# JohnLonginotto/uq

Measured on AMD Instinct MI355X. Metric: FASTQ encode MB/s (150bp synthetic; bit-exact tables vs reference), higher is better.
Workload: dtype u8

## Files before the change

uq_amd/csrc/index.hip:

```cpp
#include "common.h"
#include "swar.h"

namespace {
constexpr int IDX_THREADS = 256;
constexpr int IDX_LOADS = 4;
constexpr uint64_t IDX_WAVE_BYTES = 64 * 16 * IDX_LOADS;
constexpr uint64_t IDX_TILE = IDX_WAVE_BYTES * (IDX_THREADS / 64);
constexpr uint64_t IDX_TILE_VECS = IDX_TILE / 16;
constexpr uint32_t IDX_LIST_CAP = 1024;
constexpr uint32_t IDX_BUCKET = 1024;

__global__ __launch_bounds__(IDX_THREADS) void count_newlines_kernel(const uint4* __restrict__ abuf, uint32_t mis,
                                                                      uint64_t nbytes, uint64_t nvec,
                                                                      uint32_t* __restrict__ partials, uint16_t* __restrict__ bitmap) {
    __shared__ uint32_t lds[IDX_THREADS / 64];
    const uint32_t lane = lane_id(), w = threadIdx.x >> 6;
    const uint64_t v0 = ((uint64_t)blockIdx.x * IDX_TILE + (uint64_t)w * IDX_WAVE_BYTES) / 16 + lane;
    uint32_t c = 0;
    uint4 q[IDX_LOADS];
#pragma unroll
    for (int it = 0; it < IDX_LOADS; ++it) { const uint64_t vi = v0 + (uint64_t)it * 64; q[it] = abuf[vi < nvec ? vi : nvec - 1]; }
#pragma unroll
    for (int it = 0; it < IDX_LOADS; ++it) {
        uint64_t vi = v0 + (uint64_t)it * 64;
        int64_t p = (int64_t)(vi * 16) - (int64_t)mis;
        const uint32_t m = vi < nvec ? nl_mask16(q[it]) & valid_mask16(p, nbytes) : 0u;
        bitmap[vi] = (uint16_t)m;
        c += __popc(m);
    }
    c = wave_sum(c);
    if (lane == 0) lds[w] = c;
    __syncthreads();
    if (threadIdx.x == 0) partials[blockIdx.x] = lds[0] + lds[1] + lds[2] + lds[3];
}

#ifndef CENSUS_TPW
#define CENSUS_TPW 2
#endif
template <int TPW>
__global__ __launch_bounds__(IDX_THREADS) void census_list_kernel(const uint4* __restrict__ abuf, uint32_t mis, uint64_t nbytes, uint64_t nvec,
                                                                   uint32_t* __restrict__ partials, uint16_t* __restrict__ list,
                                                                   uint32_t* __restrict__ overflow, uint64_t tile0, uint64_t tile_end) {
    __shared__ uint32_t lds[2][IDX_THREADS / 64];
    const uint32_t lane = lane_id(), w = threadIdx.x >> 6;
    uint64_t tile = tile0 + (uint64_t)blockIdx.x * TPW;
    auto request = [&](uint64_t tl, uint4 (&q)[IDX_LOADS]) {
        const uint64_t v0 = (tl * IDX_TILE + (uint64_t)w * IDX_WAVE_BYTES) / 16 + lane;
#pragma unroll
        for (int it = 0; it < IDX_LOADS; ++it) { const uint64_t vi = v0 + (uint64_t)it * 64; q[it] = abuf[vi < nvec ? vi : nvec - 1]; }
    };
    uint4 q[IDX_LOADS];
    request(tile, q);
    bool over = false;
#pragma unroll
    for (int turn = 0; turn < TPW; ++turn, ++tile) {
        if (tile >= tile_end) break;
        uint4 qn[IDX_LOADS];
        if (turn + 1 < TPW && tile + 1 < tile_end) request(tile + 1, qn);
        const uint64_t v0 = (tile * IDX_TILE + (uint64_t)w * IDX_WAVE_BYTES) / 16 + lane;
        uint32_t m[IDX_LOADS];
#pragma unroll
        for (int it = 0; it < IDX_LOADS; ++it) {
            const uint64_t vi = v0 + (uint64_t)it * 64;
            const int64_t p = (int64_t)(vi * 16) - (int64_t)mis;
            m[it] = vi < nvec ? nl_mask16(q[it]) & valid_mask16(p, nbytes) : 0u;
        }
        const uint32_t c0 = __popc(m[0]), c1 = __popc(m[1]), c2 = __popc(m[2]), c3 = __popc(m[3]);
        const uint32_t i01 = wave_inclusive_sum(c0 | (c1 << 16)), i23 = wave_inclusive_sum(c2 | (c3 << 16));
        const uint32_t t01 = __shfl(i01, 63, 64), t23 = __shfl(i23, 63, 64);
        const uint32_t T0 = t01 & 0xFFFFu, T1 = t01 >> 16, T2 = t23 & 0xFFFFu, T3 = t23 >> 16;
        uint32_t* l = lds[turn & 1];
        if (lane == 0) l[w] = T0 + T1 + T2 + T3;
        __syncthreads();
        uint32_t base = 0, total = 0;
#pragma unroll
        for (uint32_t i = 0; i < IDX_THREADS / 64; ++i) { const uint32_t x = l[i]; if (i < w) base += x; total += x; }
        if (threadIdx.x == 0) partials[tile] = total;
        const uint32_t ex[IDX_LOADS] = {base + (i01 & 0xFFFFu) - c0, base + T0 + (i01 >> 16) - c1, base + T0 + T1 + (i23 & 0xFFFFu) - c2,
                                        base + T0 + T1 + T2 + (i23 >> 16) - c3};
        uint16_t* slot = list + tile * IDX_LIST_CAP;
#pragma unroll
        for (int it = 0; it < IDX_LOADS; ++it) {
            uint32_t mm = m[it], k = ex[it];
            const uint32_t pos0 = ((w * IDX_LOADS + it) * 64 + lane) * 16;
            while (mm) {
                const uint32_t b = (uint32_t)__ffs((int)mm) - 1u;
                mm &= mm - 1;
                if (k < IDX_LIST_CAP) slot[k] = (uint16_t)(pos0 + b); else over = true;
                ++k;
            }
        }
        if (turn + 1 < TPW) {
#pragma unroll
            for (int it = 0; it < IDX_LOADS; ++it) q[it] = qn[it];
        }
    }
    if (over) atomicOr(overflow, 1u);
}

__global__ __launch_bounds__(IDX_THREADS) void census_bucket_kernel(const uint32_t* __restrict__ partials, uint64_t nb, uint32_t* __restrict__ buckets) {
    __shared__ uint32_t lds[IDX_THREADS / 64];
    const uint64_t i0 = (uint64_t)blockIdx.x * IDX_BUCKET + (uint64_t)threadIdx.x * 4;
    uint32_t s = 0;
#pragma unroll
    for (uint32_t k = 0; k < 4; ++k) s += i0 + k < nb ? partials[i0 + k] : 0u;
    s = wave_sum(s);
    if (lane_id() == 0) lds[threadIdx.x >> 6] = s;
    __syncthreads();
    if (threadIdx.x == 0) buckets[blockIdx.x] = lds[0] + lds[1] + lds[2] + lds[3];
}
__global__ __launch_bounds__(IDX_THREADS) void census_scan_kernel(uint32_t* __restrict__ partials, uint64_t nb, const uint32_t* __restrict__ buckets,
                                                                   unsigned long long* __restrict__ d_async) {
    __shared__ uint32_t lds[IDX_THREADS / 64 + 1];
    static_assert(IDX_BUCKET == 4 * IDX_THREADS, "four counts a lane");
    const uint32_t b = blockIdx.x;
    uint32_t s = 0;
    for (uint32_t i = threadIdx.x; i < b; i += IDX_THREADS) s += buckets[i];
    s = wave_sum(s);
    if (lane_id() == 0) lds[threadIdx.x >> 6] = s;
    __syncthreads();
    uint32_t base = 0;
#pragma unroll
    for (uint32_t i = 0; i < IDX_THREADS / 64; ++i) base += lds[i];
    __syncthreads();
    const uint64_t i0 = (uint64_t)b * IDX_BUCKET + (uint64_t)threadIdx.x * 4;
    uint32_t v[4], sum = 0;
#pragma unroll
    for (uint32_t k = 0; k < 4; ++k) { v[k] = i0 + k < nb ? partials[i0 + k] : 0u; sum += v[k]; }
    uint32_t tot;
    uint32_t run = base + block_exclusive_sum<uint32_t, IDX_THREADS / 64>(sum, lds, tot);
#pragma unroll
    for (uint32_t k = 0; k < 4; ++k) { if (i0 + k < nb) partials[i0 + k] = run; run += v[k]; }
    if (b == gridDim.x - 1 && threadIdx.x == 0) d_async[0] = (unsigned long long)(base + tot);
}

__global__ void census_clear_kernel(uint32_t* __restrict__ region, uint32_t nwords, unsigned long long* __restrict__ d_async) {
    const uint32_t i = blockIdx.x * blockDim.x + threadIdx.x;
    if (i < nwords) region[i] = 0;
    if (i < 8) d_async[i] = 0;
}

constexpr uint32_t EXP_TILES = 4;
__global__ __launch_bounds__(IDX_THREADS) void expand_list_kernel(const uint16_t* __restrict__ list, uint32_t mis, const uint32_t* __restrict__ offsets,
                                                                   uint64_t nb, uint64_t nlines, uint64_t* __restrict__ line_start,
                                                                   unsigned long long* __restrict__ d_async, uint64_t cap,
                                                                   const uint32_t* __restrict__ d_over) {
    const uint32_t lane = lane_id();
    const uint64_t tile0 = ((uint64_t)blockIdx.x * (IDX_THREADS / 64) + (threadIdx.x >> 6)) * EXP_TILES;
    if (tile0 >= nb) return;
    if (d_async) nlines = d_async[0];
    if (tile0 == 0 && lane == 0) line_start[0] = 0;
    if (d_async && *d_over) { if (lane == 0) d_async[1] = 1ull; return; }
    const uint64_t tl = tile0 + lane;
    const uint64_t mine = lane <= EXP_TILES ? (tl < nb ? (uint64_t)offsets[tl] : nlines) : 0;
    for (uint32_t k = 0; k < EXP_TILES && tile0 + k < nb; ++k) {
        const uint64_t tile = tile0 + k;
        const uint64_t P = __shfl(mine, k, 64), end = __shfl(mine, k + 1, 64);
        uint32_t cnt = (uint32_t)(end - P);
        const uint16_t* slot = list + tile * IDX_LIST_CAP;
        const int64_t p0 = (int64_t)(tile * IDX_TILE) - (int64_t)mis + 1;
        if (cnt > IDX_LIST_CAP) {
            if (d_async && lane == 0) d_async[1] = 1ull;
            cnt = IDX_LIST_CAP;
        }
        if (d_async && end > cap) {
            if (lane == 0) d_async[1] = 1ull;
            for (uint32_t j = lane; j < cnt; j += 64) if (P + j + 1 <= cap) line_start[P + j + 1] = (uint64_t)(p0 + slot[j]);
            continue;
        }
        for (uint32_t j = lane; j < cnt; j += 64) line_start[P + j + 1] = (uint64_t)(p0 + slot[j]);
    }
}

__global__ __launch_bounds__(IDX_THREADS) void scatter_newlines_kernel(const uint64_t* __restrict__ bitmap, uint32_t mis,
                                                                        const uint32_t* __restrict__ offsets,
                                                                        uint64_t nlines, uint64_t* __restrict__ line_start) {
    __shared__ uint32_t lds[IDX_THREADS / 64 + 1];
    const uint64_t wi = (uint64_t)blockIdx.x * IDX_THREADS + threadIdx.x;
    uint64_t m = bitmap[wi];
    const uint32_t c = (uint32_t)__popcll(m);
    uint32_t total;
    const uint32_t ex = block_exclusive_sum<uint32_t, IDX_THREADS / 64>(c, lds, total);
    if (blockIdx.x == 0 && threadIdx.x == 0) line_start[0] = 0;
    uint64_t k = (uint64_t)offsets[blockIdx.x] + ex;
    const int64_t p = (int64_t)(wi * 64) - (int64_t)mis;
    while (m) {
        const int b = __ffsll((unsigned long long)m) - 1;
        m &= m - 1;
        if (++k <= nlines) line_start[k] = (uint64_t)(p + b + 1);
    }
}

int census_buffers(uq_ctx* ctx, uint64_t nb) {
    if (nb + 1 > ctx->idx_partials_cap) {
        UQ_CHECK_HIP(hipStreamSynchronize(ctx->stream));
        if (ctx->idx_partials) UQ_CHECK_HIP(hipFree(ctx->idx_partials));
        if (ctx->idx_bitmap) UQ_CHECK_HIP(hipFree(ctx->idx_bitmap));
        ctx->idx_partials = nullptr; ctx->idx_bitmap = nullptr; ctx->idx_partials_cap = 0;
        UQ_CHECK_HIP(hipMalloc((void**)&ctx->idx_partials, (nb + 1) * sizeof(uint32_t)));
        static_assert(IDX_TILE_VECS == IDX_LIST_CAP, "bitmap words and list entries per tile share one allocation");
        UQ_CHECK_HIP(hipMalloc((void**)&ctx->idx_bitmap, nb * IDX_TILE_VECS * sizeof(uint16_t) + 16 + ((nb + IDX_BUCKET - 1) / IDX_BUCKET) * sizeof(uint32_t)));
        ctx->idx_partials_cap = nb + 1;
    }
    return 0;
}

uint32_t* census_buckets(uq_ctx* ctx, uint64_t nb) { return (uint32_t*)(ctx->idx_bitmap + nb * IDX_TILE_VECS) + 4; }

int run_count(uq_ctx* ctx, const uint8_t* d_buf, uint64_t nbytes, uint64_t* nblocks_out, bool list_form) {
    const uint32_t mis = (uint32_t)((uintptr_t)d_buf & 15);
    const uint64_t nvec = (nbytes + mis + 15) / 16;
    const uint64_t nb = (nvec * 16 + IDX_TILE - 1) / IDX_TILE;
    UQ_REQUIRE(nb <= 0x7fffffffu, "uq_count_lines: buffer too large for one launch");
    ctx->async_buf = nullptr;
    ctx->census_begun = false;
    UQ_TRY(census_buffers(ctx, nb));
    if (list_form) {
        uint32_t* d_over = (uint32_t*)(ctx->idx_bitmap + nb * IDX_TILE_VECS);
        UQ_CHECK_HIP(hipMemsetAsync(d_over, 0, 4, ctx->stream));
        census_list_kernel<CENSUS_TPW><<<(uint32_t)((nb + CENSUS_TPW - 1) / CENSUS_TPW), IDX_THREADS, 0, ctx->stream>>>((const uint4*)(d_buf - mis), mis, nbytes, nvec, ctx->idx_partials,
                                                                         ctx->idx_bitmap, d_over, 0, nb);
    } else {
        count_newlines_kernel<<<(uint32_t)nb, IDX_THREADS, 0, ctx->stream>>>((const uint4*)(d_buf - mis), mis, nbytes, nvec, ctx->idx_partials,
                                                                            ctx->idx_bitmap);
    }
    UQ_LAUNCH_CHECK();
    *nblocks_out = nb;
    return 0;
}
}

static int finish_count(uq_ctx* ctx, const uint8_t* d_buf, uint64_t nbytes, uint64_t nb, uint64_t* h_nlines);

extern "C" int uq_count_lines(uq_ctx* ctx, const uint8_t* d_buf, uint64_t nbytes, uint64_t* h_nlines) {
    UQ_REQUIRE(ctx && h_nlines, "uq_count_lines: null argument");
    ctx->idx_buf = nullptr;
    if (nbytes == 0) { *h_nlines = 0; return 0; }
    UQ_REQUIRE(d_buf, "uq_count_lines: null buffer");
    uint64_t nb;
    UQ_TRY(run_count(ctx, d_buf, nbytes, &nb, true));
    return finish_count(ctx, d_buf, nbytes, nb, h_nlines);
}

static int finish_count(uq_ctx* ctx, const uint8_t* d_buf, uint64_t nbytes, uint64_t nb, uint64_t* h_nlines) {
    ctx->census_begun = false;
    void* scr;
    UQ_TRY(uq_scratch(ctx, 256, &scr));
    UQ_TRY(uq_scan_exclusive_u32(ctx, ctx->idx_partials, ctx->idx_partials, nb, (uint64_t*)scr));
    UQ_TRY(uq_read_back(ctx, ctx->h_pinned, scr, 8));
    UQ_TRY(uq_read_back(ctx, ctx->h_pinned + 1, ctx->idx_bitmap + nb * IDX_TILE_VECS, 4));
    UQ_CHECK_HIP(hipStreamSynchronize(ctx->stream));
    *h_nlines = ctx->h_pinned[0];
    if ((uint32_t)ctx->h_pinned[1] == 0) { ctx->idx_buf = d_buf; ctx->idx_nbytes = nbytes; ctx->idx_nlines = *h_nlines; }
    return 0;
}

extern "C" int uq_count_lines_begin(uq_ctx* ctx, const uint8_t* d_buf, uint64_t nbytes) {
    UQ_REQUIRE(ctx && (d_buf || nbytes == 0), "uq_count_lines_begin: null argument");
    ctx->census_begun = false;
    ctx->idx_buf = nullptr;
    ctx->async_buf = nullptr;
    if (nbytes == 0) return 0;
    const uint32_t mis = (uint32_t)((uintptr_t)d_buf & 15);
    const uint64_t nb = (((nbytes + mis + 15) / 16) * 16 + IDX_TILE - 1) / IDX_TILE;
    UQ_REQUIRE(nb <= 0x7fffffffu, "uq_count_lines_begin: buffer too large");
    UQ_TRY(census_buffers(ctx, nb));
    census_clear_kernel<<<1, 64, 0, ctx->stream>>>((uint32_t*)(ctx->idx_bitmap + nb * IDX_TILE_VECS), 4, ctx->d_async);
    UQ_LAUNCH_CHECK();
    ctx->census_begun = true; ctx->census_nb = nb;
    return 0;
}

extern "C" int uq_count_lines_chunk(uq_ctx* ctx, const uint8_t* d_buf, uint64_t nbytes, uint64_t first_byte, uint64_t chunk_bytes) {
    UQ_REQUIRE(ctx && d_buf, "uq_count_lines_chunk: null argument");
    if (chunk_bytes == 0) return 0;
    const uint32_t mis = (uint32_t)((uintptr_t)d_buf & 15);
    const uint64_t nvec = (nbytes + mis + 15) / 16;
    const uint64_t nb = (nvec * 16 + IDX_TILE - 1) / IDX_TILE;
    UQ_REQUIRE(first_byte + chunk_bytes <= nbytes, "uq_count_lines_chunk: chunk beyond the buffer");
    UQ_REQUIRE((first_byte + mis) % IDX_TILE == 0 || first_byte == 0, "uq_count_lines_chunk: a chunk must start on a 16 KiB tile boundary");
    UQ_REQUIRE((first_byte + chunk_bytes + mis) % IDX_TILE == 0 || first_byte + chunk_bytes == nbytes,
               "uq_count_lines_chunk: a chunk must end on a 16 KiB tile boundary or with the buffer");
    const uint64_t t0 = (first_byte + mis) / IDX_TILE, t1 = first_byte + chunk_bytes == nbytes ? nb : (first_byte + chunk_bytes + mis) / IDX_TILE;
    if (t1 <= t0) return 0;
    census_list_kernel<CENSUS_TPW><<<(uint32_t)((t1 - t0 + CENSUS_TPW - 1) / CENSUS_TPW), IDX_THREADS, 0, ctx->stream>>>((const uint4*)(d_buf - mis), mis, nbytes, nvec, ctx->idx_partials,
                                                                            ctx->idx_bitmap, (uint32_t*)(ctx->idx_bitmap + nb * IDX_TILE_VECS), t0, t1);
    UQ_LAUNCH_CHECK();
    return 0;
}

extern "C" int uq_count_lines_end(uq_ctx* ctx, const uint8_t* d_buf, uint64_t nbytes, uint64_t* h_nlines) {
    UQ_REQUIRE(ctx && h_nlines, "uq_count_lines_end: null argument");
    if (nbytes == 0) { *h_nlines = 0; return 0; }
    const uint32_t mis = (uint32_t)((uintptr_t)d_buf & 15);
    const uint64_t nb = (((nbytes + mis + 15) / 16) * 16 + IDX_TILE - 1) / IDX_TILE;
    return finish_count(ctx, d_buf, nbytes, nb, h_nlines);
}

extern "C" int uq_count_lines_end_async(uq_ctx* ctx, const uint8_t* d_buf, uint64_t nbytes) {
    UQ_REQUIRE(ctx && (d_buf || nbytes == 0), "uq_count_lines_end_async: null argument");
    ctx->idx_buf = nullptr; ctx->async_buf = nullptr; ctx->async_read = false;
    const bool begun = ctx->census_begun && nbytes != 0;
    ctx->census_begun = false;
    if (!begun) UQ_CHECK_HIP(hipMemsetAsync(ctx->d_async, 0, 64, ctx->stream));
    if (nbytes == 0) { ctx->h_pinned[8000] = 0; ctx->h_pinned[8001] = 0; ctx->h_pinned[8002] = 0; ctx->async_buf = d_buf; ctx->async_nbytes = 0; return 0; }
    const uint32_t mis = (uint32_t)((uintptr_t)d_buf & 15);
    const uint64_t nb = (((nbytes + mis + 15) / 16) * 16 + IDX_TILE - 1) / IDX_TILE;
    if (begun && ctx->census_nb == nb) {
        const uint32_t nbk = (uint32_t)((nb + IDX_BUCKET - 1) / IDX_BUCKET);
        census_bucket_kernel<<<nbk, IDX_THREADS, 0, ctx->stream>>>(ctx->idx_partials, nb, census_buckets(ctx, nb));
        UQ_LAUNCH_CHECK();
        census_scan_kernel<<<nbk, IDX_THREADS, 0, ctx->stream>>>(ctx->idx_partials, nb, census_buckets(ctx, nb), ctx->d_async);
        UQ_LAUNCH_CHECK();
    } else {
        if (begun) UQ_CHECK_HIP(hipMemsetAsync(ctx->d_async, 0, 64, ctx->stream));
        UQ_TRY(uq_scan_exclusive_u32(ctx, ctx->idx_partials, ctx->idx_partials, nb, (uint64_t*)ctx->d_async));
    }
    ctx->async_buf = d_buf; ctx->async_nbytes = nbytes;
    return 0;
}

extern "C" int uq_index_lines_async(uq_ctx* ctx, const uint8_t* d_buf, uint64_t nbytes, uint64_t capacity_lines, uint64_t* d_line_start) {
    UQ_REQUIRE(ctx && d_line_start, "uq_index_lines_async: null argument");
    UQ_REQUIRE(ctx->async_buf == d_buf && ctx->async_nbytes == nbytes, "uq_index_lines_async: not the buffer of the last uq_count_lines_end_async");
    UQ_REQUIRE(capacity_lines < (uint64_t(1) << 32), "uq_index_lines_async: more than 2^32-1 lines in one shard");
    if (nbytes == 0) { UQ_CHECK_HIP(hipMemsetAsync(d_line_start, 0, 8, ctx->stream)); return 0; }
    const uint32_t mis = (uint32_t)((uintptr_t)d_buf & 15);
    const uint64_t nb = (((nbytes + mis + 15) / 16) * 16 + IDX_TILE - 1) / IDX_TILE;
    expand_list_kernel<<<(uint32_t)((nb + EXP_TILES * (IDX_THREADS / 64) - 1) / (EXP_TILES * (IDX_THREADS / 64))), IDX_THREADS, 0, ctx->stream>>>(ctx->idx_bitmap, mis, ctx->idx_partials,
                                                                                                                 nb, 0, d_line_start, ctx->d_async, capacity_lines,
                                                                                                                 (const uint32_t*)(ctx->idx_bitmap + nb * IDX_TILE_VECS));
    UQ_LAUNCH_CHECK();
    return 0;
}

namespace {
__global__ void async_read_back_kernel(const uint32_t* __restrict__ d_async, const uint32_t* __restrict__ over, uint32_t* __restrict__ dst) {
    const uint32_t t = threadIdx.x;
    if (t < 4) dst[t] = d_async[t];
    else if (t == 4) dst[4] = *over;
}
}

bool uq_async_sources(uq_ctx* ctx, const uint32_t** d_async, const uint32_t** d_over) {
    if (!ctx->async_buf || ctx->async_nbytes == 0 || ctx->async_read) return false;
    const uint32_t mis = (uint32_t)((uintptr_t)ctx->async_buf & 15);
    const uint64_t nb = (((ctx->async_nbytes + mis + 15) / 16) * 16 + IDX_TILE - 1) / IDX_TILE;
    *d_async = (const uint32_t*)ctx->d_async; *d_over = (const uint32_t*)(ctx->idx_bitmap + nb * IDX_TILE_VECS);
    return true;
}

int uq_async_read_back(uq_ctx* ctx) {
    const uint32_t *d_async, *d_over;
    if (!uq_async_sources(ctx, &d_async, &d_over)) return 0;
    async_read_back_kernel<<<1, 64, 0, ctx->stream>>>(d_async, d_over, (uint32_t*)(ctx->d_pinned + 8000));
    UQ_LAUNCH_CHECK();
    ctx->async_read = true;
    return 0;
}

extern "C" int uq_count_lines_wait(uq_ctx* ctx, const uint8_t* d_buf, uint64_t nbytes, uint64_t* h_nlines, int* h_ok) {
    UQ_REQUIRE(ctx && h_nlines && h_ok, "uq_count_lines_wait: null argument");
    UQ_REQUIRE(ctx->async_buf == d_buf && ctx->async_nbytes == nbytes, "uq_count_lines_wait: not the buffer of the last uq_count_lines_end_async");
    *h_nlines = 0; *h_ok = 1;
    if (nbytes == 0) { ctx->async_buf = nullptr; return 0; }
    UQ_TRY(uq_async_read_back(ctx));
    ctx->async_read = false;
    ctx->async_buf = nullptr;
    UQ_CHECK_HIP(hipStreamSynchronize(ctx->stream));
    *h_nlines = ctx->h_pinned[8000];
    *h_ok = ctx->h_pinned[8001] == 0 && (uint32_t)ctx->h_pinned[8002] == 0;
    return 0;
}

extern "C" int uq_index_lines(uq_ctx* ctx, const uint8_t* d_buf, uint64_t nbytes, uint64_t nlines, uint64_t* d_line_start) {
    UQ_REQUIRE(ctx && d_line_start, "uq_index_lines: null argument");
    UQ_REQUIRE(nlines < (uint64_t(1) << 32), "uq_index_lines: more than 2^32-1 lines in one shard");
    if (nbytes == 0 || nlines == 0) {
        UQ_CHECK_HIP(hipMemsetAsync(d_line_start, 0, 8, ctx->stream));
        return 0;
    }
    uint64_t nb;
    const uint32_t mis = (uint32_t)((uintptr_t)d_buf & 15);
    const uint64_t nvec = (nbytes + mis + 15) / 16;
    if (ctx->idx_buf == d_buf && ctx->idx_nbytes == nbytes) {
        UQ_REQUIRE(ctx->idx_nlines == nlines, "uq_index_lines: nlines %llu does not match the census %llu",
                   (unsigned long long)nlines, (unsigned long long)ctx->idx_nlines);
        nb = (nvec * 16 + IDX_TILE - 1) / IDX_TILE;
        ctx->idx_buf = nullptr;
        expand_list_kernel<<<(uint32_t)((nb + EXP_TILES * (IDX_THREADS / 64) - 1) / (EXP_TILES * (IDX_THREADS / 64))), IDX_THREADS, 0, ctx->stream>>>(ctx->idx_bitmap, mis, ctx->idx_partials,
                                                                                                                     nb, nlines, d_line_start, nullptr, 0, nullptr);
        UQ_LAUNCH_CHECK();
        return 0;
    }
    UQ_TRY(run_count(ctx, d_buf, nbytes, &nb, false));
    UQ_TRY(uq_scan_exclusive_u32(ctx, ctx->idx_partials, ctx->idx_partials, nb, nullptr));
    ctx->idx_buf = nullptr;
    scatter_newlines_kernel<<<(uint32_t)nb, IDX_THREADS, 0, ctx->stream>>>((const uint64_t*)ctx->idx_bitmap, mis, ctx->idx_partials, nlines,
                                                                           d_line_start);
    UQ_LAUNCH_CHECK();
    return 0;
}
```

uq_amd/csrc/swar.h:

```cpp
#pragma once
#include "common.h"

__device__ __forceinline__ uint32_t nl_bits(uint32_t v) {
    v ^= 0x0A0A0A0Au;
    uint32_t t = (v & 0x7F7F7F7Fu) + 0x7F7F7F7Fu;
    return ~(t | v | 0x7F7F7F7Fu);
}
__device__ __forceinline__ uint32_t nl_mask16(uint4 q) {
    auto nib = [](uint32_t w) { return (((nl_bits(w) >> 7) & 0x01010101u) * 0x01020408u >> 24) & 0xFu; };
    return nib(q.x) | (nib(q.y) << 4) | (nib(q.z) << 8) | (nib(q.w) << 12);
}
__device__ __forceinline__ uint32_t valid_mask16(int64_t p, uint64_t nbytes) {
    if (p >= 0 && (uint64_t)p + 16 <= nbytes) return 0xFFFFu;
    uint32_t m = 0;
#pragma unroll
    for (int i = 0; i < 16; ++i) {
        int64_t q = p + i;
        if (q >= 0 && (uint64_t)q < nbytes) m |= 1u << i;
    }
    return m;
}

__device__ __forceinline__ void lds_window8(const uint8_t* base, int32_t o, uint32_t& lo, uint32_t& hi) {
    const uint32_t* p = (const uint32_t*)(base + (o & ~3));
    const uint32_t a = p[0], b = p[1], c = p[2];
    const uint32_t sh = (uint32_t)o & 3u;
    lo = __builtin_amdgcn_alignbyte(b, a, sh);
    hi = __builtin_amdgcn_alignbyte(c, b, sh);
}
__device__ __forceinline__ void lds_window8_at(const uint8_t* base, int32_t aligned, uint32_t sh, uint32_t& lo, uint32_t& hi) {
    const uint32_t* p = (const uint32_t*)(base + aligned);
    const uint32_t a = p[0], b = p[1], c = p[2];
    lo = __builtin_amdgcn_alignbyte(b, a, sh);
    hi = __builtin_amdgcn_alignbyte(c, b, sh);
}
__device__ __forceinline__ void window_masks(uint32_t nbad, uint32_t& mlo, uint32_t& mhi) {
    mlo = nbad >= 4 ? 0u : (0xFFFFFFFFu << (8 * nbad));
    mhi = nbad >= 8 ? 0u : (nbad > 4 ? (0xFFFFFFFFu << (8 * (nbad - 4))) : 0xFFFFFFFFu);
}
__device__ __forceinline__ uint32_t bfi(uint32_t mask, uint32_t a, uint32_t b) { return (a & mask) | (b & ~mask); }
__device__ __forceinline__ uint32_t nonzero_bytes(uint32_t x) {
    const uint32_t nz = (((x & 0x7F7F7F7Fu) + 0x7F7F7F7Fu) | x) & 0x80808080u;
    return (nz - (nz >> 7)) | nz;
}
```

Before: 1.628 million.

## Rework census list kernel: one tile per block, LDS-staged list, DPP scan

The census list kernel now handles one tile per block instead of two prefetched tiles. Loads are nontemporal with a clamped in-tile index, and newline masks come from udot4 byte packing. Per-byte validity masking is confined to edge tiles, and the wave prefix sum uses DPP. Newline positions are written as scattered 16-bit stores into an LDS image, then copied out to global memory with coalesced 16-byte stores. The aim is to cut scattered global writes and ALU work, at the cost of an extra barrier and losing the cross-tile load prefetch.

```diff
diff --git a/uq_amd/csrc/index.hip b/uq_amd/csrc/index.hip
--- a/uq_amd/csrc/index.hip
+++ b/uq_amd/csrc/index.hip
@@ -34,68 +34,79 @@
     if (threadIdx.x == 0) partials[blockIdx.x] = lds[0] + lds[1] + lds[2] + lds[3];
 }
 
-#ifndef CENSUS_TPW
-#define CENSUS_TPW 2
-#endif
-template <int TPW>
-__global__ __launch_bounds__(IDX_THREADS) void census_list_kernel(const uint4* __restrict__ abuf, uint32_t mis, uint64_t nbytes, uint64_t nvec,
-                                                                   uint32_t* __restrict__ partials, uint16_t* __restrict__ list,
-                                                                   uint32_t* __restrict__ overflow, uint64_t tile0, uint64_t tile_end) {
-    __shared__ uint32_t lds[2][IDX_THREADS / 64];
+__device__ __forceinline__ uint32_t wave_inclusive_sum_dpp(uint32_t x) {
+    int v = (int)x;
+    v += __builtin_amdgcn_update_dpp(0, v, 0x111, 0xf, 0xf, false);
+    v += __builtin_amdgcn_update_dpp(0, v, 0x112, 0xf, 0xf, false);
+    v += __builtin_amdgcn_update_dpp(0, v, 0x114, 0xf, 0xf, false);
+    v += __builtin_amdgcn_update_dpp(0, v, 0x118, 0xf, 0xf, false);
+    v += __builtin_amdgcn_update_dpp(0, v, 0x142, 0xa, 0xf, false);
+    v += __builtin_amdgcn_update_dpp(0, v, 0x143, 0xc, 0xf, false);
+    return (uint32_t)v;
+}
+
+__global__ __launch_bounds__(IDX_THREADS, 8) void census_list_kernel(const uint4* __restrict__ abuf, uint32_t mis, uint64_t nbytes, uint64_t nvec,
+                                                                      uint32_t* __restrict__ partials, uint16_t* __restrict__ list,
+                                                                      uint32_t* __restrict__ overflow, uint64_t tile0) {
+    __shared__ uint32_t lds[IDX_THREADS / 64];
+    __shared__ __attribute__((aligned(16))) uint16_t img[IDX_LIST_CAP];
     const uint32_t lane = lane_id(), w = threadIdx.x >> 6;
-    uint64_t tile = tile0 + (uint64_t)blockIdx.x * TPW;
-    auto request = [&](uint64_t tl, uint4 (&q)[IDX_LOADS]) {
-        const uint64_t v0 = (tl * IDX_TILE + (uint64_t)w * IDX_WAVE_BYTES) / 16 + lane;
-#pragma unroll
-        for (int it = 0; it < IDX_LOADS; ++it) { const uint64_t vi = v0 + (uint64_t)it * 64; q[it] = abuf[vi < nvec ? vi : nvec - 1]; }
-    };
+    const uint32_t off = w * (uint32_t)(IDX_WAVE_BYTES / 16) + lane;
+    const uint64_t tl = tile0 + blockIdx.x;
+    const char* src = (const char*)(abuf + tl * IDX_TILE_VECS);
+    const uint64_t left = nvec - tl * IDX_TILE_VECS;
+    const uint32_t last = left < IDX_TILE_VECS ? (uint32_t)left - 1u : (uint32_t)IDX_TILE_VECS - 1u;
     uint4 q[IDX_LOADS];
-    request(tile, q);
+#pragma unroll
+    for (int it = 0; it < IDX_LOADS; ++it) {
+        typedef uint32_t v4u __attribute__((ext_vector_type(4)));
+        const v4u x = __builtin_nontemporal_load((const v4u*)(src + min(off + (uint32_t)it * 64u, last) * 16u));
+        q[it] = make_uint4(x.x, x.y, x.z, x.w);
+    }
+    uint32_t m[IDX_LOADS];
+#pragma unroll
+    for (int it = 0; it < IDX_LOADS; ++it) m[it] = nl_mask16_dot(q[it]);
+    if (!((tl > 0 || mis == 0) && (tl + 1) * IDX_TILE <= nbytes + mis)) {
+        const uint64_t room = nbytes + mis - tl * IDX_TILE;
+        const int32_t lo = tl == 0 ? (int32_t)mis : 0, hi = room < IDX_TILE ? (int32_t)room : (int32_t)IDX_TILE;
+#pragma unroll
+        for (int it = 0; it < IDX_LOADS; ++it) {
+            const int32_t b = (int32_t)((off + (uint32_t)it * 64u) * 16u);
+            const int32_t nh = min(max(hi - b, 0), 16), nl = min(max(lo - b, 0), 16);
+            m[it] &= ((1u << nh) - 1u) & ~((1u << nl) - 1u);
+        }
+    }
+    const uint32_t c0 = __popc(m[0]), c1 = __popc(m[1]), c2 = __popc(m[2]), c3 = __popc(m[3]);
+    const uint32_t i01 = wave_inclusive_sum_dpp(c0 | (c1 << 16)), i23 = wave_inclusive_sum_dpp(c2 | (c3 << 16));
+    const uint32_t t01 = (uint32_t)__builtin_amdgcn_readlane((int)i01, 63), t23 = (uint32_t)__builtin_amdgcn_readlane((int)i23, 63);
+    const uint32_t T0 = t01 & 0xFFFFu, T1 = t01 >> 16, T2 = t23 & 0xFFFFu, T3 = t23 >> 16;
+    if (lane == 0) lds[w] = T0 + T1 + T2 + T3;
+    __syncthreads();
+    uint32_t base = 0, total = 0;
+#pragma unroll
+    for (uint32_t i = 0; i < IDX_THREADS / 64; ++i) { const uint32_t x = lds[i]; if (i < w) base += x; total += x; }
+    if (threadIdx.x == 0) partials[tl] = total;
+    const uint32_t ex[IDX_LOADS] = {base + (i01 & 0xFFFFu) - c0, base + T0 + (i01 >> 16) - c1, base + T0 + T1 + (i23 & 0xFFFFu) - c2,
+                                    base + T0 + T1 + T2 + (i23 >> 16) - c3};
     bool over = false;
 #pragma unroll
-    for (int turn = 0; turn < TPW; ++turn, ++tile) {
-        if (tile >= tile_end) break;
-        uint4 qn[IDX_LOADS];
-        if (turn + 1 < TPW && tile + 1 < tile_end) request(tile + 1, qn);
-        const uint64_t v0 = (tile * IDX_TILE + (uint64_t)w * IDX_WAVE_BYTES) / 16 + lane;
-        uint32_t m[IDX_LOADS];
-#pragma unroll
-        for (int it = 0; it < IDX_LOADS; ++it) {
-            const uint64_t vi = v0 + (uint64_t)it * 64;
-            const int64_t p = (int64_t)(vi * 16) - (int64_t)mis;
-            m[it] = vi < nvec ? nl_mask16(q[it]) & valid_mask16(p, nbytes) : 0u;
+    for (int it = 0; it < IDX_LOADS; ++it) {
+        uint32_t mm = m[it], k = ex[it];
+        const uint32_t pos0 = (off + (uint32_t)it * 64u) * 16u;
+        while (mm) {
+            const uint32_t b = (uint32_t)__ffs((int)mm) - 1u;
+            mm &= mm - 1;
+            if (k < IDX_LIST_CAP) img[k] = (uint16_t)(pos0 + b); else over = true;
+            ++k;
         }
-        const uint32_t c0 = __popc(m[0]), c1 = __popc(m[1]), c2 = __popc(m[2]), c3 = __popc(m[3]);
-        const uint32_t i01 = wave_inclusive_sum(c0 | (c1 << 16)), i23 = wave_inclusive_sum(c2 | (c3 << 16));
-        const uint32_t t01 = __shfl(i01, 63, 64), t23 = __shfl(i23, 63, 64);
-        const uint32_t T0 = t01 & 0xFFFFu, T1 = t01 >> 16, T2 = t23 & 0xFFFFu, T3 = t23 >> 16;
-        uint32_t* l = lds[turn & 1];
-        if (lane == 0) l[w] = T0 + T1 + T2 + T3;
-        __syncthreads();
-        uint32_t base = 0, total = 0;
-#pragma unroll
-        for (uint32_t i = 0; i < IDX_THREADS / 64; ++i) { const uint32_t x = l[i]; if (i < w) base += x; total += x; }
-        if (threadIdx.x == 0) partials[tile] = total;
-        const uint32_t ex[IDX_LOADS] = {base + (i01 & 0xFFFFu) - c0, base + T0 + (i01 >> 16) - c1, base + T0 + T1 + (i23 & 0xFFFFu) - c2,
-                                        base + T0 + T1 + T2 + (i23 >> 16) - c3};
-        uint16_t* slot = list + tile * IDX_LIST_CAP;
-#pragma unroll
-        for (int it = 0; it < IDX_LOADS; ++it) {
-            uint32_t mm = m[it], k = ex[it];
-            const uint32_t pos0 = ((w * IDX_LOADS + it) * 64 + lane) * 16;
-            while (mm) {
-                const uint32_t b = (uint32_t)__ffs((int)mm) - 1u;
-                mm &= mm - 1;
-                if (k < IDX_LIST_CAP) slot[k] = (uint16_t)(pos0 + b); else over = true;
-                ++k;
-            }
-        }
-        if (turn + 1 < TPW) {
-#pragma unroll
-            for (int it = 0; it < IDX_LOADS; ++it) q[it] = qn[it];
-        }
-    }
+    }
+    __syncthreads();
+    if (threadIdx.x * 8u < (total < IDX_LIST_CAP ? total : IDX_LIST_CAP)) ((uint4*)(list + tl * IDX_LIST_CAP))[threadIdx.x] = ((const uint4*)img)[threadIdx.x];
     if (over) atomicOr(overflow, 1u);
+}
+
+void launch_census_list(uq_ctx* ctx, const uint4* abuf, uint32_t mis, uint64_t nbytes, uint64_t nvec, uint32_t* d_over, uint64_t t0, uint64_t t1) {
+    census_list_kernel<<<(uint32_t)(t1 - t0), IDX_THREADS, 0, ctx->stream>>>(abuf, mis, nbytes, nvec, ctx->idx_partials, ctx->idx_bitmap, d_over, t0);
 }
 
 __global__ __launch_bounds__(IDX_THREADS) void census_bucket_kernel(const uint32_t* __restrict__ partials, uint64_t nb, uint32_t* __restrict__ buckets) {
@@ -218,8 +229,7 @@
     if (list_form) {
         uint32_t* d_over = (uint32_t*)(ctx->idx_bitmap + nb * IDX_TILE_VECS);
         UQ_CHECK_HIP(hipMemsetAsync(d_over, 0, 4, ctx->stream));
-        census_list_kernel<CENSUS_TPW><<<(uint32_t)((nb + CENSUS_TPW - 1) / CENSUS_TPW), IDX_THREADS, 0, ctx->stream>>>((const uint4*)(d_buf - mis), mis, nbytes, nvec, ctx->idx_partials,
-                                                                         ctx->idx_bitmap, d_over, 0, nb);
+        launch_census_list(ctx, (const uint4*)(d_buf - mis), mis, nbytes, nvec, d_over, 0, nb);
     } else {
         count_newlines_kernel<<<(uint32_t)nb, IDX_THREADS, 0, ctx->stream>>>((const uint4*)(d_buf - mis), mis, nbytes, nvec, ctx->idx_partials,
                                                                             ctx->idx_bitmap);
@@ -283,8 +293,7 @@
                "uq_count_lines_chunk: a chunk must end on a 16 KiB tile boundary or with the buffer");
     const uint64_t t0 = (first_byte + mis) / IDX_TILE, t1 = first_byte + chunk_bytes == nbytes ? nb : (first_byte + chunk_bytes + mis) / IDX_TILE;
     if (t1 <= t0) return 0;
-    census_list_kernel<CENSUS_TPW><<<(uint32_t)((t1 - t0 + CENSUS_TPW - 1) / CENSUS_TPW), IDX_THREADS, 0, ctx->stream>>>((const uint4*)(d_buf - mis), mis, nbytes, nvec, ctx->idx_partials,
-                                                                            ctx->idx_bitmap, (uint32_t*)(ctx->idx_bitmap + nb * IDX_TILE_VECS), t0, t1);
+    launch_census_list(ctx, (const uint4*)(d_buf - mis), mis, nbytes, nvec, (uint32_t*)(ctx->idx_bitmap + nb * IDX_TILE_VECS), t0, t1);
     UQ_LAUNCH_CHECK();
     return 0;
 }
diff --git a/uq_amd/csrc/swar.h b/uq_amd/csrc/swar.h
--- a/uq_amd/csrc/swar.h
+++ b/uq_amd/csrc/swar.h
@@ -9,6 +9,11 @@
 __device__ __forceinline__ uint32_t nl_mask16(uint4 q) {
     auto nib = [](uint32_t w) { return (((nl_bits(w) >> 7) & 0x01010101u) * 0x01020408u >> 24) & 0xFu; };
     return nib(q.x) | (nib(q.y) << 4) | (nib(q.z) << 8) | (nib(q.w) << 12);
+}
+__device__ __forceinline__ uint32_t nl_mask16_dot(uint4 q) {
+    const uint32_t lo = __builtin_amdgcn_udot4(nl_bits(q.y), 0x80402010u, __builtin_amdgcn_udot4(nl_bits(q.x), 0x08040201u, 0u, false), false);
+    const uint32_t hi = __builtin_amdgcn_udot4(nl_bits(q.w), 0x80402010u, __builtin_amdgcn_udot4(nl_bits(q.z), 0x08040201u, 0u, false), false);
+    return (lo >> 7) | (hi << 1);
 }
 __device__ __forceinline__ uint32_t valid_mask16(int64_t p, uint64_t nbytes) {
     if (p >= 0 && (uint64_t)p + 16 <= nbytes) return 0xFFFFu;
```

New measurement: 1.671 million, median of 6. 2.6% higher.
